# abhishekjoshi2/cuGP

Measured on AMD Instinct MI355X. Metric: GP log-lik+grad evals/sec (N=8192, D=10), higher is better.
Workload: dtype f64; 1 GPU; gp_loglik_grad_N8192_D10; experts=1, experts_per_gpu=1, overlap=True, full=False

## Files before the change

cugp_amd/capi.py:

```python
import ctypes as C
import os

import numpy as np

HERE = os.path.dirname(os.path.abspath(__file__))
LIB_PATH = os.path.join(HERE, "lib", "libcugp.so")

_dp = C.POINTER(C.c_double)
_ip = C.POINTER(C.c_int)
OBJECTIVE = C.CFUNCTYPE(None, C.c_void_p, _dp, _dp, _dp)
VALUE_FN = C.CFUNCTYPE(None, C.c_void_p, _dp, _dp)
GRADIENT_FN = C.CFUNCTYPE(None, C.c_void_p, _dp, _dp)
OBJECTIVE_N = C.CFUNCTYPE(None, C.c_void_p, _dp, C.c_int, _dp, _dp)

CUGP_OK = 0
CUGP_KERNEL_SE, CUGP_KERNEL_MATERN32, CUGP_KERNEL_MATERN52 = 0, 1, 2
CUGP_COMBINE_POE, CUGP_COMBINE_GPOE, CUGP_COMBINE_BCM, CUGP_COMBINE_RBCM = 0, 1, 2, 3
CUGP_COMBINE_REFERENCE = -1
CUGP_ERR_INVALID, CUGP_ERR_NOMEM, CUGP_ERR_DEVICE, CUGP_ERR_NODEVICE = -1, -2, -3, -4
ERR_NAMES = {-1: "CUGP_ERR_INVALID", -2: "CUGP_ERR_NOMEM", -3: "CUGP_ERR_DEVICE", -4: "CUGP_ERR_NODEVICE",
             -5: "CUGP_ERR_BUSY"}


class CugpError(RuntimeError):
# ... 129 lines not shown
    "cugp_bcm_create_split_ard_kernel": (C.c_int, [_dp, _dp, C.c_int, C.c_int, C.c_int, C.c_int, _ip, C.c_int,
                                                   C.POINTER(C.c_void_p)]),
    "cugp_bcm_num_hyper": (C.c_int, [C.c_void_p, _ip]),
    "cugp_bcm_set_loghyper_ard": (C.c_int, [C.c_void_p, _dp, C.c_int]),
    "cugp_bcm_get_loghyper_ard": (C.c_int, [C.c_void_p, _dp, C.c_int]),
    "cugp_bcm_loglik_grad_ard": (C.c_int, [C.c_void_p, _dp, _dp, C.c_int, _dp]),
    "cugp_bcm_loglik_grad_rows_ard": (C.c_int, [C.c_void_p, _dp, C.c_int]),
    "cugp_bcm_loglik_grad_rows_device_ard": (C.c_int, [C.c_void_p, C.c_void_p, _ip, C.c_int]),
    "cugp_bcm_loglik_grad_allgather_ard": (C.c_int, [C.c_void_p, C.c_void_p, C.c_int, C.c_int, _dp]),
    "cugp_bcm_cg_solve_ard": (C.c_int, [C.c_void_p, C.c_int, _dp, C.c_int, _ip]),
    "cugp_test_gemm_nt": (C.c_int, [C.c_int, C.c_int, C.c_int, _dp, _dp, _dp, C.c_int]),
    "cugp_mfma_peak_tflops": (C.c_int, [C.c_int, _dp]),
    "cugp_set_tuning": (C.c_int, [C.c_int, C.c_int]),
    "cugp_set_handle_tuning": (C.c_int, [C.c_void_p, C.c_int, C.c_int, C.c_int]),
    "cugp_get_handle_tuning": (C.c_int, [C.c_void_p, C.c_int, C.POINTER(C.c_int)]),
    "cugp_bench_la": (C.c_int, [C.c_int, C.c_int, C.c_int, C.c_int, _dp]),
    "cugp_bench_la_check": (C.c_int, [C.c_int, C.c_int, C.c_int, C.c_int, _dp, _dp]),
    "cugp_potrf_plan": (C.c_int, [C.c_int, C.c_int, C.c_int, C.c_int, _ip]),
    "cugp_potrf_plan_sub": (C.c_int, [C.c_int, C.c_int, C.c_int, C.c_int, C.c_int, _ip]),
}

_lib = None


def _share_torch_hip_runtime():
    import importlib.util
    import sys
    if "torch" in sys.modules or os.environ.get("CUGP_OWN_HIP_RUNTIME", "0") not in ("", "0"):
        return
    try:
# ... 43 lines not shown
```

cugp_amd/csrc/bcm.cpp:

```cpp
#include <cmath>
#include <cstdio>
#include <cstring>
#include <new>
#include <vector>

#include "../../include/cugp.h"
#include <hip/hip_runtime.h>

#include "group.h"

struct DeviceSet {
    int device = 0;
    std::vector<int> idx;
    cugp_group* group = nullptr;
    bool grouped_now = false;
    Scratch grad_rows;
    hipStream_t grad_stream = nullptr;
    std::vector<hipEvent_t> ev;
};

struct cugp_bcm {
    std::vector<DeviceSet> sets;
    std::vector<cugp_gp*> experts;
    std::vector<int> rows;
// ... 92 lines not shown
        if (rows[k] <= 0) { delete b; return CUGP_ERR_INVALID; }
        nmax = rows[k] > nmax ? rows[k] : nmax;
        nmin = rows[k] < nmin ? rows[k] : nmin;
    }
    const int tmax = (nmax + 127) / 128, tmin = (nmin + 127) / 128;
    const int pad_to = (tmax - tmin <= (tmin / 16 > 1 ? tmin / 16 : 1)) ? nmax : 0;
    const int nsets = ndev < nexperts ? ndev : nexperts;
    b->sets.resize(nsets);
    for (int s = 0; s < nsets; s++) b->sets[s].device = devices[s];
    for (int k = 0; k < nexperts; k++) {
        DeviceSet& ds = b->sets[k % nsets];
        cugp_gp* g = nullptr;
        int rc = ard ? cugp_create_ard_kernel(rows[k], d, ds.device, pad_to, kernel, &g)
                     : cugp_create_kernel(rows[k], d, ds.device, pad_to, kernel, &g);
        if (rc) { cugp_bcm_destroy(b); return rc; }
        cugp_mark_bcm_expert(g);
        if (nexperts > nsets) cugp_set_overlap(g, 0);
        b->experts.push_back(g);
        b->rows.push_back(rows[k]);
        ds.idx.push_back(k);
    }
    for (DeviceSet& ds : b->sets) {
        if (ds.idx.size() < 2 && !(nexperts > nsets)) continue;
        std::vector<cugp_gp*> mine;
        for (int k : ds.idx) mine.push_back(b->experts[k]);
        if (cugp_group_create(mine.data(), (int)mine.size(), &ds.group) != CUGP_OK) ds.group = nullptr;
    }
    *out = b;
    return CUGP_OK;
}

int bcm_create_split(const double* X, const double* y, int N, int D, int K, int ndev, const int* devices, int kernel,
                     bool ard, cugp_bcm** out)
// ... 796 lines not shown
```

cugp_amd/csrc/cugp_capi.cpp:

```cpp
#include <hip/hip_runtime.h>

#include <algorithm>
#include <atomic>
#include <cmath>
#include <cstdio>
#include <cstdlib>
#include <cstdint>
#include <cstring>
#include <mutex>
#include <string>
#include <vector>

#include "../../include/cugp.h"
#include "group.h"
#include "kernels.h"

using namespace cugp;

namespace {

thread_local std::string g_err;

int fail(int code, const char* what, hipError_t e = hipSuccess)
{
// ... 51 lines not shown
    unsigned* tickets = nullptr;
    double* dout = nullptr;
    double* hout = nullptr;
    int row = 8;
    double* hrows = nullptr;
    bool overlap = false;
    int gcap = 0;
};

struct cugp_gp {
    int n = 0, d = 0, npad = 0, nt = 0, device = 0;
    hipStream_t stream = nullptr;
    hipStream_t aux = nullptr;
    hipStream_t aux2 = nullptr;
    hipStream_t lq = nullptr;
    std::vector<hipEvent_t> bev;
    std::vector<hipEvent_t> oev;
    std::vector<hipEvent_t> lev;
    double *dX = nullptr, *dy = nullptr, *dA = nullptr, *dT = nullptr, *dU = nullptr, *dKinv = nullptr;
    double *dz = nullptr, *dalpha = nullptr, *dw = nullptr, *d16 = nullptr, *dlogdet = nullptr, *dpart = nullptr, *d64 = nullptr;
    double* dout = nullptr;
    unsigned* dtickets = nullptr;
    double* hout = nullptr;
    int nblocks_trace = 0;
    bool ard = false;
    int nh = 3;
    std::vector<double> theta = {0, 0, 0}, last_g = {NAN, NAN, NAN};
    int kernel = KERNEL_SE;
    bool have_data = false;
    bool factor_valid = false;
// ... 219 lines not shown
{
    if (g->bar_quota > 0) g_bar_used[g->device >= 0 && g->device < 64 ? g->device : 63].fetch_sub(g->bar_quota, std::memory_order_relaxed);
    g->bar_quota = -1;
}
int barrier_cap(cugp_gp* g)
{
    if (g->grp) return g->grp->gcap;
    const int share = barrier_share(g);
    return g->overlap && share >= 16 ? share / 2 : share;
}

int pipe_block(const cugp_gp* g, bool with_inverse)
{
    const bool overlap = g->grp ? g->grp->overlap : g->overlap;
    int w = (with_inverse && overlap) ? g->tune[TUNE_PIPE_BLOCK] : 0;
    if (w < 0) w = g->nt <= 8 ? 1 : ((g->nt + 8) / 16 > 2 ? (g->nt + 8) / 16 : 2);
    return w >= g->nt ? 0 : w;
}

struct TimedLaunch {
    cugp_gp* g; hipStream_t s; bool on, ext;
    TimedLaunch(cugp_gp* g_, hipStream_t s_, bool want, bool chain = false)
        : g(g_), s(s_), on(want && g_->kev_used + 2 <= (int)g_->kev.size()), ext(g_->prof >= 4)
    {
        if (!on) { if (chain) g->last_main = -1; return; }
        g->kev_prev[g->kev_used / 2] = chain ? g->last_main : -1;
        if (chain) g->last_main = g->kev_used / 2;
        if (g->prof >= 5) stamp_next_launch(g->dstamps + g->kev_used / 2);
        else if (ext) time_next_launch(g->kev[g->kev_used], g->kev[g->kev_used + 1]);
        else if (hipEventRecord(g->kev[g->kev_used], s) != hipSuccess) on = false;
    }
    ~TimedLaunch() { if (on && ext && timing_pending()) { time_next_launch(nullptr, nullptr); stamp_next_launch(nullptr); } }
// ... 584 lines not shown
    g->kernel = kernel;
    if (ard) { g->nh = d + 2; g->theta.assign(g->nh, 0.0); g->last_g.assign(g->nh, NAN); }
    const size_t nrow = ard ? (size_t)ARD_ROW_GRAD + g->nh : 8, ncol = g->nh;
    g->nt = ((n > npad_min ? n : npad_min) + TILE - 1) / TILE;
    g->npad = g->nt * TILE;
    g->nblocks_trace = trace_num_blocks(g->npad);
    *out = nullptr;
    {
        std::lock_guard<std::mutex> lk(g_tune_mu);
        tune_defaults_locked();
        for (int k = 0; k < TUNE_COUNT; k++) g->tune[k] = g_tune_default[k];
    }
    g_live[device < 64 ? device : 63].fetch_add(1, std::memory_order_relaxed);
    g->counted = true;
    hipError_t e = hipSetDevice(device);
    int plo = 0, phi = 0;
    if (e == hipSuccess && g->tune[TUNE_STREAM_PRIO] != 0) e = hipDeviceGetStreamPriorityRange(&plo, &phi);
    const int pmain = (g->tune[TUNE_STREAM_PRIO] & 1) ? phi : 0, pinv = (g->tune[TUNE_STREAM_PRIO] & 2) ? plo : 0;
    auto mkstream = [&](hipStream_t* s, int prio) {
        return g->tune[TUNE_STREAM_PRIO] != 0 ? hipStreamCreateWithPriority(s, hipStreamNonBlocking, prio)
                                             : hipStreamCreateWithFlags(s, hipStreamNonBlocking);
    };
    if (e == hipSuccess) e = mkstream(&g->stream, pmain);
    if (e == hipSuccess) e = mkstream(&g->aux, pinv);
    if (e == hipSuccess) e = mkstream(&g->aux2, pinv);
    if (e == hipSuccess) e = mkstream(&g->lq, pinv);
    for (std::vector<hipEvent_t>* v : {&g->bev, &g->oev, &g->lev}) {
        v->assign((size_t)g->nt + 2, nullptr);
        for (size_t i = 0; i < v->size() && e == hipSuccess; i++) e = hipEventCreateWithFlags(&(*v)[i], hipEventDisableTiming);
    }
    if (e == hipSuccess) e = hipMalloc((void**)&g->dX, (size_t)n * d * sizeof(double));
    if (e == hipSuccess) e = hipMalloc((void**)&g->dy, (size_t)g->npad * sizeof(double));
    if (e == hipSuccess) e = hipMalloc((void**)&g->dz, (size_t)g->npad * sizeof(double));
    if (e == hipSuccess) e = hipMalloc((void**)&g->dalpha, (size_t)g->npad * sizeof(double));
    if (e == hipSuccess) e = hipMalloc((void**)&g->dw, (size_t)g->npad * sizeof(double));
    if (e == hipSuccess) e = hipMalloc((void**)&g->d16, (size_t)g->nt * 8 * 256 * sizeof(double));
    if (e == hipSuccess) e = hipMalloc((void**)&g->d64, (size_t)g->nt * 8192 * sizeof(double));
    if (e == hipSuccess) e = hipMalloc((void**)&g->dlogdet, (size_t)g->nt * sizeof(double));
    if (e == hipSuccess) e = hipMalloc((void**)&g->dpart, (size_t)g->nblocks_trace * ncol * sizeof(double));
    if (e == hipSuccess) e = hipMalloc((void**)&g->dout, nrow * sizeof(double));
    if (e == hipSuccess) e = hipMalloc((void**)&g->dtickets, (size_t)ticket_count(g->nt) * sizeof(unsigned));
// ... 49 lines not shown
    for (hipEvent_t e : g->kev) (void)hipEventDestroy(e);
    for (std::vector<hipEvent_t>* v : {&g->bev, &g->oev, &g->lev})
        for (hipEvent_t e : *v)
            if (e) (void)hipEventDestroy(e);
    if (g->aux) (void)hipStreamDestroy(g->aux);
    if (g->aux2) (void)hipStreamDestroy(g->aux2);
    if (g->lq) (void)hipStreamDestroy(g->lq);
    if (g->stream) (void)hipStreamDestroy(g->stream);
    delete g;
    return CUGP_OK;
}

int cugp_set_overlap(cugp_gp* g, int enable)
{
    if (!g) return CUGP_ERR_INVALID;
    g->overlap = enable != 0;
    return CUGP_OK;
}

int cugp_dims(const cugp_gp* g, int* n, int* d, int* npad)
{
    if (!g) return CUGP_ERR_INVALID;
    if (n) *n = g->n;
    if (d) *d = g->d;
    if (npad) *npad = g->npad;
    return CUGP_OK;
}

static int set_data_common(cugp_gp* g, const double* X, const double* y, hipMemcpyKind kind)
{
    if (!g || !X || !y) return fail(CUGP_ERR_INVALID, "cugp_set_data: null argument");
    int rc;
    if ((rc = use_device(g))) return rc;
    if ((rc = fetch_eval(g))) return rc;
    HIPCHK(hipMemcpyAsync(g->dX, X, (size_t)g->n * g->d * sizeof(double), kind, g->stream));
    HIPCHK(hipMemsetAsync(g->dy, 0, (size_t)g->npad * sizeof(double), g->stream));
    HIPCHK(hipMemcpyAsync(g->dy, y, (size_t)g->n * sizeof(double), kind, g->stream));
    HIPCHK(hipStreamSynchronize(g->stream));
    g->have_data = true;
    g->factor_valid = g->inverse_valid = false;
    return CUGP_OK;
}

int cugp_set_data(cugp_gp* g, const double* X, const double* y) { return set_data_common(g, X, y, hipMemcpyHostToDevice); }

int cugp_set_data_device(cugp_gp* g, const double* dX, const double* dy)
{
    return set_data_common(g, dX, dy, hipMemcpyDeviceToDevice);
}
// ... 422 lines not shown

static int cov_factor_handle(cugp_gp* g, int tiles)
{
    int rc;
    if (!g->cov_f || g->cov_tiles < tiles) {
        HIPCHK(hipStreamSynchronize(g->stream));
        if (g->cov_f) (void)cugp_destroy(g->cov_f);
        g->cov_f = nullptr;
        g->cov_tiles = 0;
        cugp_gp* f = nullptr;
        if ((rc = cugp_create(tiles * TILE, 1, g->device, &f))) return rc;
        g_live[f->device < 64 ? f->device : 63].fetch_sub(1, std::memory_order_relaxed);
        f->counted = false;
        f->overlap = false;
        f->is_factor = true;
        if ((rc = ensure_factor_bufs(f))) { cugp_destroy(f); return rc; }
        g->cov_f = f;
        g->cov_tiles = tiles;
        if ((rc = use_device(g))) return rc;
    }
    return CUGP_OK;
}

static int predict_cov_device(cugp_gp* g, const double* Xt, int nt, bool with_noise, double jitter, double** dmean,
                              cugp_gp** fout)
{
    PredBufs pb;
    int rc;
    if ((rc = predict_device(g, Xt, nt, &pb))) return rc;
    TuneScope ts(g);
    const int tiles = (nt + TILE - 1) / TILE, ntpad = tiles * TILE;
// ... 209 lines not shown
    launch_trace(g->dX, g->n, d, g->npad, cf, g->dKinv, g->dalpha, g->dpart, s, {}, g->dz, g->dlogdet, g->dout, g->hout,
                 g->dtickets + 2 * g->nt);
    hipError_t e = hipGetLastError();
    if (e == hipSuccess) e = hipStreamSynchronize(s);
    if (e != hipSuccess) { (void)hipStreamSynchronize(s); return fail(CUGP_ERR_DEVICE, "cugp_append", e); }
    g->pev_valid = false;
    (void)read_result_row(g, g->hout, true);
    if (!std::isfinite(g->last_ll)) discard_eval(g);
    return CUGP_OK;
}

int cugp_mark_bcm_expert(cugp_gp* g)
{
    if (!g) return CUGP_ERR_INVALID;
    g->bcm_expert = true;
    return CUGP_OK;
}

int cugp_compute_K_train(cugp_gp* g, double* K)
{
    if (!g || !K) return CUGP_ERR_INVALID;
    if (!g->have_data) return fail(CUGP_ERR_INVALID, "no training data set");
    int rc;
    if ((rc = use_device(g))) return rc;
    if ((rc = fetch_eval(g))) return rc;
    if ((rc = ensure(&g->dA, (size_t)g->npad * g->npad))) return rc;
    g->factor_valid = g->inverse_valid = false;
    TuneScope ts(g);
    CovFn cf;
    if ((rc = cov_fn(g, g->stream, nullptr, &cf))) return rc;
    launch_kbuild(g->dX, g->n, g->d, g->npad, cf, g->dA, true, g->stream);
// ... 1010 lines not shown
    tune_defaults_locked();
    g_tune_default[key] = value;
    return CUGP_OK;
}

int cugp_set_handle_tuning(cugp_gp* g, int key, int value, int own)
{
    if (!g || key < 0 || key >= TUNE_COUNT) return CUGP_ERR_INVALID;
    int rc;
    if ((rc = fetch_eval(g))) return rc;
    g->tune_own[key] = own != 0;
    if (own && g->tune[key] != value) {
        g->tune[key] = value;
        if (key != TUNE_GRAPHS) g->cfg_epoch++;
    }
    return CUGP_OK;
}

int cugp_get_handle_tuning(cugp_gp* g, int key, int* value)
{
    if (!g || !value || key < 0 || key >= TUNE_COUNT) return CUGP_ERR_INVALID;
    sync_tuning(g);
    *value = g->tune[key];
    return CUGP_OK;
}

int cugp_potrf_plan(int nt, int P, int near, int kb, int out[5])
{
    int v[6];
    const int rc = cugp_potrf_plan_sub(nt, P, near, 1, kb, v);
    if (rc || !out) return rc ? rc : CUGP_ERR_INVALID;
// ... 139 lines not shown
    if (!experts || k <= 0 || !out) return CUGP_ERR_INVALID;
    for (int i = 0; i < k; i++)
        if (!experts[i] || experts[i]->npad != experts[0]->npad || experts[i]->d != experts[0]->d ||
            experts[i]->device != experts[0]->device)
            return CUGP_ERR_INVALID;
    for (int i = 0; i < k; i++)
        if (experts[i]->kernel != experts[0]->kernel)
            return fail(CUGP_ERR_INVALID, "cugp_group_create: the experts have different kernel kinds (one launch serves them all)");
    for (int i = 0; i < k; i++)
        if (experts[i]->ard != experts[0]->ard)
            return fail(CUGP_ERR_INVALID, "cugp_group_create: ARD and isotropic handles in one group (the experts of a group are all ARD or all isotropic)");
    cugp_group* gr = new (std::nothrow) cugp_group;
    if (!gr) return fail(CUGP_ERR_NOMEM, "host allocation");
    gr->experts.assign(experts, experts + k);
    for (cugp_gp* x : gr->experts) x->groups++;
    const int nt = experts[0]->nt;
    const bool ard = experts[0]->ard;
    const size_t row = ard ? (size_t)ARD_ROW_GRAD + experts[0]->nh : 8;
    gr->ctx.row = (int)row;
    hipError_t e = hipSetDevice(experts[0]->device);
    if (e == hipSuccess) e = hipMalloc((void**)&gr->dtab, (size_t)k * sizeof(ExpertPtrs));
    if (e == hipSuccess) e = hipMalloc((void**)&gr->ctx.tickets, (size_t)k * ticket_count(nt) * sizeof(unsigned));
    if (e == hipSuccess) e = hipMalloc((void**)&gr->ctx.dout, (size_t)k * row * sizeof(double));
    if (e == hipSuccess) e = hipHostMalloc((void**)&gr->ctx.hout, (size_t)k * 8 * sizeof(double), hipHostMallocDefault);
    if (e == hipSuccess) memset(gr->ctx.hout, 0, (size_t)k * 8 * sizeof(double));
    if (e == hipSuccess && ard) e = hipHostMalloc((void**)&gr->ctx.hrows, (size_t)k * row * sizeof(double), hipHostMallocDefault);
    if (e == hipSuccess && ard) memset(gr->ctx.hrows, 0, (size_t)k * row * sizeof(double));
    if (e != hipSuccess) {
        cugp_group_destroy(gr);
        return fail(e == hipErrorOutOfMemory ? CUGP_ERR_NOMEM : CUGP_ERR_DEVICE, "cugp_group_create", e);
// ... 254 lines not shown
```

cugp_amd/csrc/kernels.h:

```cpp
#pragma once
#ifndef CUGP_HOST_EMUL
#include <hip/hip_runtime.h>
#endif

namespace cugp {

constexpr int TILE = 128;

enum { TUNE_LAUUM_WM2_MAX = 0,
       TUNE_TRTRI_WM2_MAX = 1,
       TUNE_SYRK_REM_MAX = 2,
       TUNE_PIPE_BLOCK = 3,
       TUNE_BORDER_WM2_MAX = 4,
       TUNE_GRAPHS = 5,
       TUNE_GROUP_OVERLAP = 6,
       TUNE_GROUP_MAX_TILES = 7,
       TUNE_PANEL = 8,
       TUNE_NEAR_TILES = 9,
       TUNE_PANEL_MIN_NT = 10,
       TUNE_LAUUM_STREAM = 11,
       TUNE_FINALIZE_FUSE_MAX = 12,
       TUNE_SPLIT_REM_MAX = 13,
       TUNE_STEP_QUARTER_MAX = 14,
       TUNE_STREAM_PRIO = 15,
       TUNE_BARRIER_SPIN = 16,
       TUNE_SUBPANEL = 17,
       TUNE_ZFUSE = 18,
       TUNE_PRED_CHUNK = 19,
       TUNE_COV_SPLIT = 20,
       TUNE_COUNT = 21 };
extern const int g_tune_init[TUNE_COUNT];
extern thread_local const int* t_tune;
inline int tune(int key) { return t_tune[key]; }

enum { KERNEL_SE = 0, KERNEL_MATERN32 = 1, KERNEL_MATERN52 = 2, KERNEL_COUNT = 3 };

struct ExpertPtrs {
    double *A, *T, *U, *Kinv, *d16, *d64, *logdet, *y, *z, *alpha, *w, *part, *out;
    const double* X;
    unsigned* tickets;
    int n;
};
struct Batch {
    const ExpertPtrs* tab = nullptr;
    int count = 1;
// ... 154 lines not shown
```

cugp_amd/csrc/kernels.hip:

```cpp
#include "kernels.h"

#include <hip/hip_runtime.h>
#include <hip/hip_ext.h>

#include <cassert>
#include <cstdlib>

namespace cugp {

typedef double d4 __attribute__((ext_vector_type(4)));
typedef double d2 __attribute__((ext_vector_type(2)));

template <class T>
__device__ __forceinline__ T* GP(T* p)
{
    return (T*)(__attribute__((address_space(1))) T*)(unsigned long long)p;
}

#ifdef CUGP_WGTIMES
constexpr unsigned WGT_CAP = 1u << 19;
__device__ unsigned long long g_wgt[4 * WGT_CAP];
__device__ unsigned g_wgt_n;
struct WgTimer {
    unsigned long long t0, c0, tag;
// ... 426 lines not shown
                                                         int c0, int c1, int nfull, const ExpertPtrs* __restrict__ bt,
                                                         unsigned long long* stamp)
{
    LaunchStamp stamp_(stamp);
    if (bt) { L = GP(bt[blockIdx.y].A); T = GP(bt[blockIdx.y].T); U = GP(bt[blockIdx.y].U); }
    extern __shared__ __attribute__((aligned(16))) char smem[];
    WGT(wgt_, WGT_BORDER, a * 4 + step);
    if (WM == 2) {
        border_tile<2>(L, T, U, ld, a, w, step, c0, c1, blockIdx.x >> 2, blockIdx.x & 3, smem);
    } else if ((int)blockIdx.x < nfull) {
        border_tile<4>(L, T, U, ld, a, w, step, c0, c1, blockIdx.x, 0, smem);
    } else {
        const int y = blockIdx.x - nfull;
        border_tile<2>(L, T, U, ld, a, w, step, c0, c1, nfull + (y >> 2), y & 3, smem);
    }
}

__global__ __launch_bounds__(256, 2) void k_predict_gemm(const double* __restrict__ Ks, const double* __restrict__ T,
                                                         double* __restrict__ W, int ld, int ntt64, int n64,
                                                         unsigned long long* stamp, const ExpertPtrs* __restrict__ bt)
{
    LaunchStamp stamp_(stamp);
    if (bt) {
        const size_t off = (size_t)blockIdx.y * ntt64 * 64 * ld;
        T = GP(bt[blockIdx.y].T); Ks += off; W += off;
    }
    extern __shared__ __attribute__((aligned(16))) char smem[];
    const int tt = blockIdx.x % ntt64, p = blockIdx.x / ntt64;
#pragma unroll 1
    for (int h = 0; h < 2; h++) {
// ... 1101 lines not shown
        tile_accum_store<-1>(A + (size_t)i0 * ld + j0, ld, acc);
        return;
    }
    const int xg = blockIdx.x & 7;
    const int xq = nfull >> 3, xr = nfull & 7;
    const int tlin = (xg < xr ? xg * (xq + 1) : xr * (xq + 1) + (xg - xr) * xq) + (blockIdx.x >> 3);
    int ti, tj;
    trap_index(rev ? nfull - 1 - tlin : tlin, cb - ca, ti, tj);
    const int i0 = (ca + ti) * TILE, j0 = (ca + tj) * TILE;
    d4 acc[4][4];
    acc_zero(acc);
    tile_nt<false>(A + (size_t)i0 * ld, ld, A + (size_t)j0 * ld, ld, k0 * TILE, (k0 + kw) * TILE, acc, smem);
    tile_accum_store<-1>(A + (size_t)i0 * ld + j0, ld, acc);
}

__device__ __forceinline__ void trtri_diag_body(const double* __restrict__ A, int ld, int b,
                                                const double* __restrict__ d64, double* __restrict__ T,
                                                double* __restrict__ U, double* __restrict__ sm)
{
    const int t = threadIdx.x, wave = t >> 6;
    const double* Ab = A + (size_t)b * TILE * ld + b * TILE;
    const double* T00 = d64 + (size_t)b * 8192;
    const double* T11 = T00 + 4096;
    {
        const int r = t >> 4, c = t & 15;
        double v[NLT];
#pragma unroll
        for (int bi = 0; bi < NMT; bi++)
#pragma unroll
            for (int bj = 0; bj <= bi; bj++) {
// ... 810 lines not shown
void stamp_next_launch(unsigned long long* slot) { t_stamp = slot; }
bool timing_pending() { return t_ev0 != nullptr || t_stamp != nullptr; }
static inline unsigned long long* take_stamp() { unsigned long long* p = t_stamp; t_stamp = nullptr; return p; }
#define CUGP_LAUNCH(kernel, grid, block, lds, stream, ...)                                          \
    do {                                                                                            \
        if (t_ev0) {                                                                                \
            hipEvent_t e0_ = t_ev0, e1_ = t_ev1;                                                    \
            t_ev0 = t_ev1 = nullptr;                                                                \
            hipExtLaunchKernelGGL(kernel, grid, block, lds, stream, e0_, e1_, 0, __VA_ARGS__);      \
        } else {                                                                                    \
            hipLaunchKernelGGL(kernel, grid, block, lds, stream, __VA_ARGS__);                      \
        }                                                                                           \
    } while (0)

const int g_tune_init[TUNE_COUNT] = {768, 1200, 384, -1, 511, 1, 1, 1 << 20, 16, 500, 32, 1, 2100, 256, 1536, 0, 1 << 21, 1, 1, 0,
                                      1024};
thread_local const int* t_tune = g_tune_init;

static inline int tri_count(int n) { return n * (n + 1) / 2; }

static inline bool is_ard(const CovFn& cf)
{
    assert(!cf.ard || cf.hd);
    return cf.ard;
}

#define CUGP_COV_KERNEL(cf, stem)                                                                        \
    (is_ard(cf) ? ((cf).kind == KERNEL_MATERN32   ? stem<true, KERNEL_MATERN32>                          \
                   : (cf).kind == KERNEL_MATERN52 ? stem<true, KERNEL_MATERN52> : stem<true, KERNEL_SE>) \
                : ((cf).kind == KERNEL_MATERN32   ? stem<false, KERNEL_MATERN32>                         \
                   : (cf).kind == KERNEL_MATERN52 ? stem<false, KERNEL_MATERN52> : stem<false, KERNEL_SE>))
// ... 29 lines not shown
    int dev = 0;
    if (hipGetDevice(&dev) != hipSuccess || dev < 0 || dev > 63) dev = 63;
    if (g_attr_done >> dev & 1ull) return;
    hipError_t e = hipSuccess;
    auto attr = [&](const void* f, int bytes) {
        const hipError_t r = hipFuncSetAttribute(f, hipFuncAttributeMaxDynamicSharedMemorySize, bytes);
        if (r != hipSuccess && e == hipSuccess) e = r;
    };
    attr((const void*)k_potf2, POTF2_LDS);
    attr((const void*)k_syrk_step, STEP_LDS);
    attr((const void*)k_syrk_wide, GEMM_LDS);
    const void* gemm4[] = {(const void*)k_trtri_level<4>, (const void*)k_trtri_border<4>, (const void*)k_lauum<4>,
                           (const void*)k_test_gemm, (const void*)k_predict_cov<4>, (const void*)k_loo_product<4>,
                           (const void*)k_sparse_gram};
    for (const void* f : gemm4) attr(f, GEMM_LDS);
    attr((const void*)k_trtri_diag, TRTRI_LDS);
    attr((const void*)k_trtri_block, TRTRI_BLOCK_LDS);
    attr((const void*)k_trsm_inv64, TRSM_LDS);
    if (e != hipSuccess) { g_attr_err = e; return; }
    g_attr_done |= 1ull << dev;
}

int prepare_kernels() { set_big_lds(); return (int)g_attr_err; }

void launch_potf2(double* A, int ld, int kb, double* d16, double* d64, double* logdet_part, hipStream_t s, Batch bt)
{
    set_big_lds();
    hipLaunchKernelGGL(k_potf2, dim3(1, bt.count), dim3(256), POTF2_LDS, s, A, ld, kb, d16, d64, logdet_part, bt.tab);
}

// ... 58 lines not shown
    const int vec0 = NDIAGWG + nfull + 4 * (ntl - nfull);
    const unsigned nwg = vec0 + (zv ? m : 0);
    if (ks < 0 || ks > kb) ks = kb;
    if (kb + 1 - ks > SUBPANEL_MAX) return;
    CUGP_LAUNCH(k_syrk_step, bt.tab ? dim3(bt.count, nwg) : dim3(nwg), dim3(256), STEP_LDS, s, A, ld, kb, d16,
                       d64, logdet_part, tickets, nfull, wcol, ks, bt.tab, take_stamp(), vec0, zv, wv);
}

int launch_syrk_wide(double* A, int ld, int nt, int k0, int kw, int ca, int cb, int rev, hipStream_t s, Batch bt)
{
    if (cb > nt) cb = nt;
    if (ca >= cb || kw <= 0) return 0;
    set_big_lds();
    const int ntiles = trap_count(nt - ca, cb - ca);
    const int nfull = split_round(ntiles, bt.count);
    CUGP_LAUNCH(k_syrk_wide, dim3(nfull + 4 * (ntiles - nfull), bt.count), dim3(256), GEMM_LDS, s, A, ld, k0, kw, ca,
                       cb, ntiles, nfull, rev, bt.tab, take_stamp());
    return ntiles;
}

int launch_trtri_level(const double* L, double* T, double* U, int ld, int nt, int s, int step, hipStream_t st,
                       Batch bt, size_t off)
{
    int tiles = 0;
    for (int a0 = 0; a0 + s < nt; a0 += 2 * s) {
        int sb = nt - (a0 + s);
        if (sb > s) sb = s;
        tiles += s * sb;
    }
    if (tiles <= 0) return 0;
// ... 8 lines not shown
    return 4;
}

int launch_trtri_border1(const double* L, double* T, double* U, int ld, int ra, int rw, int c0, int c1,
                         hipStream_t st, Batch bt)
{
    const int tiles = c1 * rw;
    if (tiles <= 0) return 0;
    set_big_lds();
    if (tiles * bt.count <= tune(TUNE_BORDER_WM2_MAX)) {
        CUGP_LAUNCH(k_trtri_border<2>, dim3(tiles * 4, bt.count), dim3(256), Geo<2>::LDS, st, L, T, U, ld, ra, rw,
                           1, c0, c1, 0, bt.tab, take_stamp());
        return 2;
    }
    const int nfull = split_round(tiles, bt.count);
    CUGP_LAUNCH(k_trtri_border<4>, dim3(nfull + 4 * (tiles - nfull), bt.count), dim3(256), GEMM_LDS, st, L, T,
                       U, ld, ra, rw, 1, c0, c1, nfull, bt.tab, take_stamp());
    return 4;
}

int launch_trtri_border2(const double* L, double* T, double* U, int ld, int a, int w, hipStream_t st, Batch bt)
{
    const int tiles = a * w;
    if (tiles <= 0) return 0;
    set_big_lds();
    if (tiles * bt.count <= tune(TUNE_TRTRI_WM2_MAX)) {
        CUGP_LAUNCH(k_trtri_border<2>, dim3(tiles * 4, bt.count), dim3(256), Geo<2>::LDS, st, L, T, U, ld, a, w, 2,
                           0, 0, 0, bt.tab, take_stamp());
        return 2;
    }
    const int nfull = split_round(tiles, bt.count);
    CUGP_LAUNCH(k_trtri_border<4>, dim3(nfull + 4 * (tiles - nfull), bt.count), dim3(256), GEMM_LDS, st, L, T,
                       U, ld, a, w, 2, 0, 0, nfull, bt.tab, take_stamp());
    return 4;
}

int launch_lauum(const double* U, double* Kinv, int ld, int a, int w, hipStream_t s, Batch bt)
{
    set_big_lds();
    const int tiles = tri_count(a + w);
    if (tiles * bt.count <= tune(TUNE_LAUUM_WM2_MAX)) {
        CUGP_LAUNCH(k_lauum<2>, dim3(tiles * 4, bt.count), dim3(256), Geo<2>::LDS, s, U, Kinv, ld, a, w, 0, bt.tab, take_stamp());
        return 2;
    } else {
        const int nfull = a > 0 ? split_round(tiles, bt.count) : tiles;
        CUGP_LAUNCH(k_lauum<4>, dim3(nfull + 4 * (tiles - nfull), bt.count), dim3(256), GEMM_LDS, s, U, Kinv, ld,
                           a, w, nfull, bt.tab, take_stamp());
        return 4;
    }
}

void launch_predict_gemm(const double* Ks, const double* T, double* W, int ld, int ntt, int nt, hipStream_t s,
                         Batch bt)
{
    set_big_lds();
    CUGP_LAUNCH(k_predict_gemm, dim3(2 * ntt * nt, bt.count), dim3(256), Geo<2>::LDS, s, Ks, T, W, ld, 2 * ntt, 2 * nt,
                take_stamp(), bt.tab);
}

CovShape predict_cov_shape(int ntpad, int n)
// ... 381 lines not shown
```

cugp_amd/gp.py:

```python
import ctypes as C
import math

import numpy as np

from . import capi
from .capi import check, f64, ptr


KERNELS = {"se": capi.CUGP_KERNEL_SE, "matern32": capi.CUGP_KERNEL_MATERN32, "matern52": capi.CUGP_KERNEL_MATERN52}
KERNEL_NAMES = {v: k for k, v in KERNELS.items()}
ARD_KERNELS = {"matern32_ard": capi.CUGP_KERNEL_MATERN32, "matern52_ard": capi.CUGP_KERNEL_MATERN52}


COMBINE = {"poe": capi.CUGP_COMBINE_POE, "gpoe": capi.CUGP_COMBINE_GPOE, "bcm": capi.CUGP_COMBINE_BCM,
           "rbcm": capi.CUGP_COMBINE_RBCM}


def combine_mode(combine):
    if not isinstance(combine, str) or combine.lower() not in COMBINE:
        raise ValueError("combine must be None or one of %s, not %r" % (sorted(COMBINE), combine))
    return COMBINE[combine.lower()]


def prior_scalars(hp):
# ... 337 lines not shown
        return tr[: ne.value]

    def set_profiling(self, level):
        check(capi.lib().cugp_set_profiling(self._h, int(level)))

    def set_overlap(self, enable):
        check(capi.lib().cugp_set_overlap(self._h, 1 if enable else 0))

    def set_tuning(self, key, value, own=True):
        check(capi.lib().cugp_set_handle_tuning(self._h, int(key), int(value), 1 if own else 0))

    def get_tuning(self, key):
        v = C.c_int()
        check(capi.lib().cugp_get_handle_tuning(self._h, int(key), C.byref(v)))
        return v.value

    def phase_ms(self):
        ms = np.empty(6)
        check(capi.lib().cugp_get_phase_ms(self._h, ptr(ms)))
        return dict(zip(("kbuild", "potrf", "trtri", "lauum", "tail", "total"), ms.tolist()))

    def kernel_stats(self, reset=False, kind=0):
        s, n, f, dms = C.c_double(), C.c_longlong(), C.c_double(), C.c_double()
        check(capi.lib().cugp_get_kernel_stats_dispatch_ms(self._h, int(kind), C.byref(dms)))
        check(capi.lib().cugp_get_kernel_stats_kind(self._h, int(kind), C.byref(s), C.byref(n), C.byref(f),
                                                    1 if reset else 0))
        return {"sum_ms": s.value, "launches": n.value, "flop": f.value, "disp_ms": dms.value}


class SparseGP:
# ... 485 lines not shown
```

include/cugp.h:

```cpp
#ifndef CUGP_H
#define CUGP_H

#ifdef __cplusplus
extern "C" {
#endif

#define CUGP_OK 0
#define CUGP_ERR_INVALID (-1)
#define CUGP_ERR_NOMEM (-2)
#define CUGP_ERR_DEVICE (-3)
#define CUGP_ERR_NODEVICE (-4)
#define CUGP_ERR_BUSY (-5)

typedef struct cugp_gp cugp_gp;
typedef struct cugp_bcm cugp_bcm;

int cugp_version(void);
const char *cugp_build_id(void);
const char *cugp_last_error(void);
int cugp_device_count(int *count);

int cugp_create(int n, int d, int device, cugp_gp **out);
int cugp_create_padded(int n, int d, int device, int npad_min, cugp_gp **out);
int cugp_destroy(cugp_gp *gp);
// ... 170 lines not shown
int cugp_bcm_set_loghyper_ard(cugp_bcm *b, const double *hp, int nh);
int cugp_bcm_get_loghyper_ard(const cugp_bcm *b, double *hp, int nh);
int cugp_bcm_loglik_grad_ard(cugp_bcm *b, double *ll, double *g, int nh, double *per_expert_ll );
int cugp_bcm_loglik_grad_rows_ard(cugp_bcm *b, double *rows, int nh);
int cugp_bcm_loglik_grad_rows_device_ard(cugp_bcm *b, double *dev_rows, const int *slot, int nh);
int cugp_bcm_loglik_grad_allgather_ard(cugp_bcm *b, cugp_comm *c, int per, int nh, double *rows_out);
int cugp_bcm_cg_solve_ard(cugp_bcm *b, int budget, double *trace, int trace_cap, int *nevals);

int cugp_test_gemm_nt(int m, int n, int k, const double *A, const double *B, double *C, int device);
int cugp_mfma_peak_tflops(int device, double *tflops);
int cugp_bench_la(int op, int n, int device, int reps, double *ms);
int cugp_bench_la_check(int op, int n, int device, int reps, double *ms, double *logdet);
int cugp_set_tuning(int key, int value);
int cugp_set_handle_tuning(cugp_gp *gp, int key, int value, int own);
int cugp_get_handle_tuning(cugp_gp *gp, int key, int *value);
int cugp_potrf_plan(int nt, int P, int near_tiles, int kb, int out[5]);
int cugp_potrf_plan_sub(int nt, int P, int near_tiles, int S, int kb, int out[6]);

#ifdef __cplusplus
}
#endif
#endif
```

Baseline: 91.58 evals/s.

## Prioritize the factor chain stream and widen the inverse pipeline block for single GPs

Stream creation moves into a reusable apply_stream_prio helper. For a standalone overlapped GP with at least 64 tiles, the main (factorization) stream now gets high priority by default, and streams are recreated whenever overlap, the expert role or the tuning changes. The default pipeline block width for non-grouped GPs now comes from cugp_pipe_block_for, which gives larger blocks for big tile counts. The change also adds 512-thread, 8-wave variants of the syrk, trtri-border and lauum kernels behind TUNE_WAVES8, which is off by default. The aim is to keep the critical Cholesky chain ahead of the overlapped inverse work, at the cost of recreating streams and possibly starving the inverse work.

```diff
diff --git a/cugp_amd/capi.py b/cugp_amd/capi.py
--- a/cugp_amd/capi.py
+++ b/cugp_amd/capi.py
@@ -167,6 +167,8 @@
     "cugp_set_tuning": (C.c_int, [C.c_int, C.c_int]),
     "cugp_set_handle_tuning": (C.c_int, [C.c_void_p, C.c_int, C.c_int, C.c_int]),
     "cugp_get_handle_tuning": (C.c_int, [C.c_void_p, C.c_int, C.POINTER(C.c_int)]),
+    "cugp_chain_first": (C.c_int, [C.c_void_p, _ip]),
+    "cugp_pipe_block_for": (C.c_int, [C.c_int]),
     "cugp_bench_la": (C.c_int, [C.c_int, C.c_int, C.c_int, C.c_int, _dp]),
     "cugp_bench_la_check": (C.c_int, [C.c_int, C.c_int, C.c_int, C.c_int, _dp, _dp]),
     "cugp_potrf_plan": (C.c_int, [C.c_int, C.c_int, C.c_int, C.c_int, _ip]),
diff --git a/cugp_amd/csrc/bcm.cpp b/cugp_amd/csrc/bcm.cpp
--- a/cugp_amd/csrc/bcm.cpp
+++ b/cugp_amd/csrc/bcm.cpp
@@ -130,9 +130,10 @@
         int rc = ard ? cugp_create_ard_kernel(rows[k], d, ds.device, pad_to, kernel, &g)
                      : cugp_create_kernel(rows[k], d, ds.device, pad_to, kernel, &g);
         if (rc) { cugp_bcm_destroy(b); return rc; }
-        cugp_mark_bcm_expert(g);
-        if (nexperts > nsets) cugp_set_overlap(g, 0);
         b->experts.push_back(g);
+        rc = cugp_mark_bcm_expert(g);
+        if (!rc && nexperts > nsets) rc = cugp_set_overlap(g, 0);
+        if (rc) { cugp_bcm_destroy(b); return rc; }
         b->rows.push_back(rows[k]);
         ds.idx.push_back(k);
     }
diff --git a/cugp_amd/csrc/cugp_capi.cpp b/cugp_amd/csrc/cugp_capi.cpp
--- a/cugp_amd/csrc/cugp_capi.cpp
+++ b/cugp_amd/csrc/cugp_capi.cpp
@@ -89,6 +89,8 @@
     hipStream_t aux = nullptr;
     hipStream_t aux2 = nullptr;
     hipStream_t lq = nullptr;
+    int prio_main = 0, prio_inv = 0;
+    bool chain_first = false;
     std::vector<hipEvent_t> bev;
     std::vector<hipEvent_t> oev;
     std::vector<hipEvent_t> lev;
@@ -338,8 +340,51 @@
 {
     const bool overlap = g->grp ? g->grp->overlap : g->overlap;
     int w = (with_inverse && overlap) ? g->tune[TUNE_PIPE_BLOCK] : 0;
-    if (w < 0) w = g->nt <= 8 ? 1 : ((g->nt + 8) / 16 > 2 ? (g->nt + 8) / 16 : 2);
+    if (w < 0) w = !g->grp && !g->bcm_expert ? cugp_pipe_block_for(g->nt)
+                                            : g->nt <= 8 ? 1 : ((g->nt + 8) / 16 > 2 ? (g->nt + 8) / 16 : 2);
     return w >= g->nt ? 0 : w;
+}
+
+bool want_chain_first(const cugp_gp* g)
+{
+    const int v = g->tune[TUNE_STREAM_PRIO];
+    if (v != 0) return (v & 4) == 0 && (v & 1) != 0;
+    return !g->bcm_expert && g->groups == 0 && !g->is_factor && g->overlap && g->tune[TUNE_PIPE_BLOCK] != 0 &&
+           g->nt >= g->tune[TUNE_PRIO_MIN_NT];
+}
+
+int apply_stream_prio(cugp_gp* g)
+{
+    const int v = g->tune[TUNE_STREAM_PRIO];
+    const bool first = want_chain_first(g), inv_low = (v & 4) == 0 && (v & 2) != 0;
+    int plo = 0, phi = 0;
+    if (first || inv_low) HIPCHK(hipDeviceGetStreamPriorityRange(&plo, &phi));
+    const int pmain = first ? phi : 0, pinv = inv_low ? plo : 0;
+    hipStream_t* const all[4] = {&g->stream, &g->aux, &g->aux2, &g->lq};
+    if (g->stream && pmain == g->prio_main && pinv == g->prio_inv) return CUGP_OK;
+    hipStream_t fresh[4] = {nullptr, nullptr, nullptr, nullptr};
+    hipError_t e = hipSuccess;
+    for (int i = 0; i < 4 && e == hipSuccess; i++) {
+        const int p = i == 0 ? pmain : pinv;
+        e = pmain == 0 && pinv == 0 ? hipStreamCreateWithFlags(&fresh[i], hipStreamNonBlocking)
+                                    : hipStreamCreateWithPriority(&fresh[i], hipStreamNonBlocking, p);
+    }
+    for (int i = 0; i < 4 && e == hipSuccess; i++)
+        if (*all[i]) e = hipStreamSynchronize(*all[i]);
+    if (e != hipSuccess) {
+        for (hipStream_t s : fresh)
+            if (s) (void)hipStreamDestroy(s);
+        return fail(CUGP_ERR_DEVICE, "apply_stream_prio: the handle keeps the streams it had", e);
+    }
+    for (int i = 0; i < 4; i++) {
+        if (*all[i]) (void)hipStreamDestroy(*all[i]);
+        *all[i] = fresh[i];
+    }
+    g->prio_main = pmain;
+    g->prio_inv = pinv;
+    g->chain_first = first;
+    g->cfg_epoch++;
+    return CUGP_OK;
 }
 
 struct TimedLaunch {
@@ -954,17 +999,7 @@
     g_live[device < 64 ? device : 63].fetch_add(1, std::memory_order_relaxed);
     g->counted = true;
     hipError_t e = hipSetDevice(device);
-    int plo = 0, phi = 0;
-    if (e == hipSuccess && g->tune[TUNE_STREAM_PRIO] != 0) e = hipDeviceGetStreamPriorityRange(&plo, &phi);
-    const int pmain = (g->tune[TUNE_STREAM_PRIO] & 1) ? phi : 0, pinv = (g->tune[TUNE_STREAM_PRIO] & 2) ? plo : 0;
-    auto mkstream = [&](hipStream_t* s, int prio) {
-        return g->tune[TUNE_STREAM_PRIO] != 0 ? hipStreamCreateWithPriority(s, hipStreamNonBlocking, prio)
-                                             : hipStreamCreateWithFlags(s, hipStreamNonBlocking);
-    };
-    if (e == hipSuccess) e = mkstream(&g->stream, pmain);
-    if (e == hipSuccess) e = mkstream(&g->aux, pinv);
-    if (e == hipSuccess) e = mkstream(&g->aux2, pinv);
-    if (e == hipSuccess) e = mkstream(&g->lq, pinv);
+    if (e == hipSuccess && apply_stream_prio(g) != CUGP_OK) e = hipErrorUnknown;
     for (std::vector<hipEvent_t>* v : {&g->bev, &g->oev, &g->lev}) {
         v->assign((size_t)g->nt + 2, nullptr);
         for (size_t i = 0; i < v->size() && e == hipSuccess; i++) e = hipEventCreateWithFlags(&(*v)[i], hipEventDisableTiming);
@@ -1044,8 +1079,10 @@
 int cugp_set_overlap(cugp_gp* g, int enable)
 {
     if (!g) return CUGP_ERR_INVALID;
+    int rc;
+    if ((rc = use_device(g)) || (rc = fetch_eval(g))) return rc;
     g->overlap = enable != 0;
-    return CUGP_OK;
+    return apply_stream_prio(g);
 }
 
 int cugp_dims(const cugp_gp* g, int* n, int* d, int* npad)
@@ -1063,6 +1100,8 @@
     int rc;
     if ((rc = use_device(g))) return rc;
     if ((rc = fetch_eval(g))) return rc;
+    sync_tuning(g);
+    if ((rc = apply_stream_prio(g))) return rc;
     HIPCHK(hipMemcpyAsync(g->dX, X, (size_t)g->n * g->d * sizeof(double), kind, g->stream));
     HIPCHK(hipMemsetAsync(g->dy, 0, (size_t)g->npad * sizeof(double), g->stream));
     HIPCHK(hipMemcpyAsync(g->dy, y, (size_t)g->n * sizeof(double), kind, g->stream));
@@ -1515,7 +1554,7 @@
         f->counted = false;
         f->overlap = false;
         f->is_factor = true;
-        if ((rc = ensure_factor_bufs(f))) { cugp_destroy(f); return rc; }
+        if ((rc = apply_stream_prio(f)) || (rc = ensure_factor_bufs(f))) { cugp_destroy(f); return rc; }
         g->cov_f = f;
         g->cov_tiles = tiles;
         if ((rc = use_device(g))) return rc;
@@ -1755,7 +1794,9 @@
 {
     if (!g) return CUGP_ERR_INVALID;
     g->bcm_expert = true;
-    return CUGP_OK;
+    int rc;
+    if ((rc = use_device(g)) || (rc = fetch_eval(g))) return rc;
+    return apply_stream_prio(g);
 }
 
 int cugp_compute_K_train(cugp_gp* g, double* K)
@@ -2796,7 +2837,27 @@
         g->tune[key] = value;
         if (key != TUNE_GRAPHS) g->cfg_epoch++;
     }
-    return CUGP_OK;
+    if (key != TUNE_STREAM_PRIO && key != TUNE_PRIO_MIN_NT && key != TUNE_PIPE_BLOCK) return CUGP_OK;
+    if (!own) sync_tuning(g);
+    if ((rc = use_device(g))) return rc;
+    return apply_stream_prio(g);
+}
+
+int cugp_chain_first(const cugp_gp* g, int* on)
+{
+    if (!g || !on) return fail(CUGP_ERR_INVALID, "cugp_chain_first: null argument");
+    *on = g->chain_first ? 1 : 0;
+    return CUGP_OK;
+}
+
+int cugp_pipe_block_for(int nt)
+{
+    if (nt <= 8) return 1;
+    int w = (nt + 8) / 16;
+    if (w < 2) w = 2;
+    if (nt >= 60 && w < 5) w = 5;
+    if (nt >= 72 && w < 8) w = 8;
+    return w > 16 ? 16 : w;
 }
 
 int cugp_get_handle_tuning(cugp_gp* g, int key, int* value)
@@ -2966,6 +3027,11 @@
     if (!gr) return fail(CUGP_ERR_NOMEM, "host allocation");
     gr->experts.assign(experts, experts + k);
     for (cugp_gp* x : gr->experts) x->groups++;
+    for (cugp_gp* x : gr->experts)
+        if (hipSetDevice(x->device) != hipSuccess || fetch_eval(x) != CUGP_OK || apply_stream_prio(x) != CUGP_OK) {
+            cugp_group_destroy(gr);
+            return fail(CUGP_ERR_DEVICE, "cugp_group_create: the experts' streams");
+        }
     const int nt = experts[0]->nt;
     const bool ard = experts[0]->ard;
     const size_t row = ard ? (size_t)ARD_ROW_GRAD + experts[0]->nh : 8;
diff --git a/cugp_amd/csrc/kernels.h b/cugp_amd/csrc/kernels.h
--- a/cugp_amd/csrc/kernels.h
+++ b/cugp_amd/csrc/kernels.h
@@ -28,7 +28,9 @@
        TUNE_ZFUSE = 18,
        TUNE_PRED_CHUNK = 19,
        TUNE_COV_SPLIT = 20,
-       TUNE_COUNT = 21 };
+       TUNE_PRIO_MIN_NT = 21,
+       TUNE_WAVES8 = 22,
+       TUNE_COUNT = 23 };
 extern const int g_tune_init[TUNE_COUNT];
 extern thread_local const int* t_tune;
 inline int tune(int key) { return t_tune[key]; }
diff --git a/cugp_amd/csrc/kernels.hip b/cugp_amd/csrc/kernels.hip
--- a/cugp_amd/csrc/kernels.hip
+++ b/cugp_amd/csrc/kernels.hip
@@ -464,6 +464,165 @@
         const int y = blockIdx.x - nfull;
         border_tile<2>(L, T, U, ld, a, w, step, c0, c1, nfull + (y >> 2), y & 3, smem);
     }
+}
+
+template <bool NEGA>
+__device__ __forceinline__ void tile_nt8(const double* __restrict__ Ag, int lda, const double* __restrict__ Bg, int ldb,
+                                         int kbeg, int kend, d4 (&acc)[2][4], char* smem)
+{
+    typedef Geo<4> G;
+    const int t = opaque_tid();
+    const int lane = t & 63, wave = t >> 6;
+    const int wr = wave >> 1, wc = wave & 1;
+    const int srow = t >> 3, skp = t & 7;
+    const double* ag = Ag + (size_t)srow * lda + 2 * skp;
+    const double* bg = Bg + (size_t)srow * ldb + 2 * skp;
+    d2 ra[2], rb[2];
+    int wa[2], wb[2];
+#pragma unroll
+    for (int q = 0; q < 2; q++) {
+        wa[q] = skp * G::PLANE + (srow + 64 * q) * 16;
+        wb[q] = G::OPER + skp * G::PLANE + bpos<4>(srow + 64 * q) * 16;
+    }
+    const int fr = lane & 15, fk = lane >> 4;
+    const int abase = (fk >> 1) * G::PLANE + (wr * 32 + fr) * 16 + (fk & 1) * 8;
+    const int bbase = G::OPER + (fk >> 1) * G::PLANE + (wc * 64 + fr) * 16 + (fk & 1) * 8;
+    const int nk = (kend - kbeg) / BK;
+    if (nk <= 0) return;
+#pragma unroll
+    for (int q = 0; q < 2; q++) {
+        ra[q] = *(const d2*)(ag + (size_t)(64 * q) * lda + kbeg);
+        rb[q] = *(const d2*)(bg + (size_t)(64 * q) * ldb + kbeg);
+    }
+#pragma unroll
+    for (int q = 0; q < 2; q++) {
+        *(d2*)(smem + wa[q]) = NEGA ? -ra[q] : ra[q];
+        *(d2*)(smem + wb[q]) = rb[q];
+    }
+    __syncthreads();
+#define CUGP_STAGE8(HALF, MORE, KNEXT)                                                              \
+    do {                                                                                            \
+        const char* cur_ = smem + (HALF) * G::STAGE;                                                \
+        char* nxt_ = smem + (1 - (HALF)) * G::STAGE;                                                \
+        const bool more_ = (MORE);                                                                  \
+        if (more_) {                                                                                \
+            const int k_ = (KNEXT);                                                                 \
+            _Pragma("unroll") for (int q = 0; q < 2; q++) {                                         \
+                ra[q] = *(const d2*)(ag + (size_t)(64 * q) * lda + k_);                             \
+                rb[q] = *(const d2*)(bg + (size_t)(64 * q) * ldb + k_);                             \
+            }                                                                                       \
+        }                                                                                           \
+        _Pragma("unroll") for (int kk = 0; kk < BK / 4; kk++) {                                     \
+            double a[2], b[4];                                                                      \
+            _Pragma("unroll") for (int m = 0; m < 2; m++) a[m] = *(const double*)(cur_ + abase + kk * 2 * G::PLANE + m * 256); \
+            _Pragma("unroll") for (int n = 0; n < 4; n++) b[n] = *(const double*)(cur_ + bbase + kk * 2 * G::PLANE + n * 256); \
+            _Pragma("unroll") for (int m = 0; m < 2; m++)                                           \
+                _Pragma("unroll") for (int n = 0; n < 4; n++)                                       \
+                    acc[m][n] = __builtin_amdgcn_mfma_f64_16x16x4f64(a[m], b[n], acc[m][n], 0, 0, 0); \
+        }                                                                                           \
+        if (more_) {                                                                                \
+            _Pragma("unroll") for (int q = 0; q < 2; q++) {                                         \
+                *(d2*)(nxt_ + wa[q]) = NEGA ? -ra[q] : ra[q];                                       \
+                *(d2*)(nxt_ + wb[q]) = rb[q];                                                       \
+            }                                                                                       \
+        }                                                                                           \
+        __syncthreads();                                                                            \
+    } while (0)
+    int kt = 0;
+    for (; kt + 1 < nk; kt += 2) {
+        CUGP_STAGE8(0, true, kbeg + (kt + 1) * BK);
+        CUGP_STAGE8(1, kt + 2 < nk, kbeg + (kt + 2) * BK);
+    }
+    if (kt < nk) CUGP_STAGE8(0, false, 0);
+#undef CUGP_STAGE8
+}
+
+template <int SIGN>
+__device__ __forceinline__ void tile_out8(double* __restrict__ C, int ldc, const d4 (&acc)[2][4])
+{
+    const int tid = opaque_tid();
+    const int lane = tid & 63, wave = tid >> 6;
+    const int wr = wave >> 1, wc = wave & 1;
+#pragma unroll
+    for (int m = 0; m < 2; m++) {
+        double* const c0 = C + (size_t)(wr * 32 + m * 16 + (lane >> 4)) * ldc + wc * 64 + 2 * (lane & 15);
+        d2 v[4][2];
+        if (SIGN != 0) {
+#pragma unroll
+            for (int r = 0; r < 4; r++)
+#pragma unroll
+                for (int np = 0; np < 2; np++) v[r][np] = *(const d2*)(c0 + (size_t)(4 * r) * ldc + np * 32);
+        }
+#pragma unroll
+        for (int r = 0; r < 4; r++)
+#pragma unroll
+            for (int np = 0; np < 2; np++) {
+                d2* dst = (d2*)(c0 + (size_t)(4 * r) * ldc + np * 32);
+                if (SIGN == 0) *dst = (d2){acc[m][2 * np][r], acc[m][2 * np + 1][r]};
+                else if (SIGN > 0) *dst = (d2){v[r][np][0] + acc[m][2 * np][r], v[r][np][1] + acc[m][2 * np + 1][r]};
+                else *dst = (d2){v[r][np][0] - acc[m][2 * np][r], v[r][np][1] - acc[m][2 * np + 1][r]};
+            }
+    }
+}
+
+__device__ __forceinline__ void acc_zero8(d4 (&acc)[2][4])
+{
+#pragma unroll
+    for (int m = 0; m < 2; m++)
+#pragma unroll
+        for (int n = 0; n < 4; n++) acc[m][n] = (d4){0.0, 0.0, 0.0, 0.0};
+}
+
+__global__ __launch_bounds__(512, 4) void k_lauum8(const double* __restrict__ U, double* __restrict__ Kinv, int ld, int a,
+                                                   int w, const ExpertPtrs* __restrict__ bt, unsigned long long* stamp)
+{
+    LaunchStamp stamp_(stamp);
+    if (bt) { U = GP(bt[blockIdx.y].U); Kinv = GP(bt[blockIdx.y].Kinv); }
+    extern __shared__ __attribute__((aligned(16))) char smem[];
+    int ti, tj;
+    tri_index(blockIdx.x, ti, tj);
+    double* C = Kinv + (size_t)(ti * TILE) * ld + tj * TILE;
+    d4 acc[2][4];
+    acc_zero8(acc);
+    tile_nt8<false>(U + (size_t)(ti * TILE) * ld, ld, U + (size_t)(tj * TILE) * ld, ld, (ti < a ? a : ti) * TILE,
+                    (a + w) * TILE, acc, smem);
+    if (ti < a) tile_out8<1>(C, ld, acc);
+    else tile_out8<0>(C, ld, acc);
+}
+
+__global__ __launch_bounds__(256, 2) void k_lauum_rest(const double* __restrict__ U, double* __restrict__ Kinv, int ld,
+                                                       int a, int w, int x0, const ExpertPtrs* __restrict__ bt)
+{
+    if (bt) { U = GP(bt[blockIdx.y].U); Kinv = GP(bt[blockIdx.y].Kinv); }
+    extern __shared__ __attribute__((aligned(16))) char smem[];
+    lauum_tile<2>(U, Kinv, ld, a, w, x0 + (blockIdx.x >> 2), blockIdx.x & 3, smem);
+}
+
+__global__ __launch_bounds__(512, 4) void k_trtri_border8(const double* __restrict__ L, double* __restrict__ T,
+                                                          const double* __restrict__ U, int ld, int a, int w, int c0,
+                                                          int c1, const ExpertPtrs* __restrict__ bt,
+                                                          unsigned long long* stamp)
+{
+    LaunchStamp stamp_(stamp);
+    if (bt) { L = GP(bt[blockIdx.y].A); T = GP(bt[blockIdx.y].T); U = GP(bt[blockIdx.y].U); }
+    extern __shared__ __attribute__((aligned(16))) char smem[];
+    const int tj = blockIdx.x / w, ti = a + blockIdx.x % w;
+    double* W = T + (size_t)(tj * TILE) * ld + ti * TILE;
+    d4 acc[2][4];
+    acc_zero8(acc);
+    tile_nt8<false>(U + (size_t)(tj * TILE) * ld, ld, L + (size_t)(ti * TILE) * ld, ld, (tj > c0 ? tj : c0) * TILE,
+                    c1 * TILE, acc, smem);
+    if (tj < c0) tile_out8<1>(W, ld, acc);
+    else tile_out8<0>(W, ld, acc);
+}
+
+__global__ __launch_bounds__(256, 2) void k_trtri_border_rest(const double* __restrict__ L, double* __restrict__ T,
+                                                              double* __restrict__ U, int ld, int a, int w, int c0,
+                                                              int c1, int x0, const ExpertPtrs* __restrict__ bt)
+{
+    if (bt) { L = GP(bt[blockIdx.y].A); T = GP(bt[blockIdx.y].T); U = GP(bt[blockIdx.y].U); }
+    extern __shared__ __attribute__((aligned(16))) char smem[];
+    border_tile<2>(L, T, U, ld, a, w, 1, c0, c1, x0 + (blockIdx.x >> 2), blockIdx.x & 3, smem);
 }
 
 __global__ __launch_bounds__(256, 2) void k_predict_gemm(const double* __restrict__ Ks, const double* __restrict__ T,
@@ -1595,6 +1754,43 @@
     tile_accum_store<-1>(A + (size_t)i0 * ld + j0, ld, acc);
 }
 
+__global__ __launch_bounds__(512, 4) void k_syrk_wide8(double* __restrict__ A, int ld, int k0, int kw, int ca, int cb,
+                                                       int rev, const ExpertPtrs* __restrict__ bt,
+                                                       unsigned long long* stamp)
+{
+    LaunchStamp stamp_(stamp);
+    if (bt) A = GP(bt[blockIdx.y].A);
+    extern __shared__ __attribute__((aligned(16))) char smem[];
+    __builtin_amdgcn_s_setprio(1);
+    const int nfull = gridDim.x;
+    const int xg = blockIdx.x & 7;
+    const int xq = nfull >> 3, xr = nfull & 7;
+    const int tlin = (xg < xr ? xg * (xq + 1) : xr * (xq + 1) + (xg - xr) * xq) + (blockIdx.x >> 3);
+    int ti, tj;
+    trap_index(rev ? nfull - 1 - tlin : tlin, cb - ca, ti, tj);
+    const int i0 = (ca + ti) * TILE, j0 = (ca + tj) * TILE;
+    d4 acc[2][4];
+    acc_zero8(acc);
+    tile_nt8<false>(A + (size_t)i0 * ld, ld, A + (size_t)j0 * ld, ld, k0 * TILE, (k0 + kw) * TILE, acc, smem);
+    tile_out8<-1>(A + (size_t)i0 * ld + j0, ld, acc);
+}
+
+__global__ __launch_bounds__(256, 2) void k_syrk_wide_rest(double* __restrict__ A, int ld, int k0, int kw, int ca, int cb,
+                                                           int x0, const ExpertPtrs* __restrict__ bt)
+{
+    if (bt) A = GP(bt[blockIdx.y].A);
+    extern __shared__ __attribute__((aligned(16))) char smem[];
+    __builtin_amdgcn_s_setprio(1);
+    const int y = blockIdx.x;
+    int ti, tj;
+    trap_index(x0 + (y >> 2), cb - ca, ti, tj);
+    const int i0 = (ca + ti) * TILE + ((y >> 1) & 1) * 64, j0 = (ca + tj) * TILE + (y & 1) * 64;
+    d4 acc[2][2];
+    acc_zero(acc);
+    tile_nt<false>(A + (size_t)i0 * ld, ld, A + (size_t)j0 * ld, ld, k0 * TILE, (k0 + kw) * TILE, acc, smem);
+    tile_accum_store<-1>(A + (size_t)i0 * ld + j0, ld, acc);
+}
+
 __device__ __forceinline__ void trtri_diag_body(const double* __restrict__ A, int ld, int b,
                                                 const double* __restrict__ d64, double* __restrict__ T,
                                                 double* __restrict__ U, double* __restrict__ sm)
@@ -2435,7 +2631,7 @@
     } while (0)
 
 const int g_tune_init[TUNE_COUNT] = {768, 1200, 384, -1, 511, 1, 1, 1 << 20, 16, 500, 32, 1, 2100, 256, 1536, 0, 1 << 21, 1, 1, 0,
-                                      1024};
+                                      1024, 64, 0};
 thread_local const int* t_tune = g_tune_init;
 
 static inline int tri_count(int n) { return n * (n + 1) / 2; }
@@ -2495,6 +2691,7 @@
                            (const void*)k_test_gemm, (const void*)k_predict_cov<4>, (const void*)k_loo_product<4>,
                            (const void*)k_sparse_gram};
     for (const void* f : gemm4) attr(f, GEMM_LDS);
+    for (const void* f : {(const void*)k_syrk_wide8, (const void*)k_lauum8, (const void*)k_trtri_border8}) attr(f, GEMM_LDS);
     attr((const void*)k_trtri_diag, TRTRI_LDS);
     attr((const void*)k_trtri_block, TRTRI_BLOCK_LDS);
     attr((const void*)k_trsm_inv64, TRSM_LDS);
@@ -2583,6 +2780,14 @@
     set_big_lds();
     const int ntiles = trap_count(nt - ca, cb - ca);
     const int nfull = split_round(ntiles, bt.count);
+    if (tune(TUNE_WAVES8) != 0 && nfull > 0) {
+        CUGP_LAUNCH(k_syrk_wide8, dim3(nfull, bt.count), dim3(512), GEMM_LDS, s, A, ld, k0, kw, ca, cb, rev, bt.tab,
+                    take_stamp());
+        if (ntiles > nfull)
+            hipLaunchKernelGGL(k_syrk_wide_rest, dim3(4 * (ntiles - nfull), bt.count), dim3(256), Geo<2>::LDS, s, A, ld, k0,
+                               kw, ca, cb, nfull, bt.tab);
+        return ntiles;
+    }
     CUGP_LAUNCH(k_syrk_wide, dim3(nfull + 4 * (ntiles - nfull), bt.count), dim3(256), GEMM_LDS, s, A, ld, k0, kw, ca,
                        cb, ntiles, nfull, rev, bt.tab, take_stamp());
     return ntiles;
@@ -2621,6 +2826,14 @@
         return 2;
     }
     const int nfull = split_round(tiles, bt.count);
+    if (tune(TUNE_WAVES8) != 0 && nfull > 0) {
+        CUGP_LAUNCH(k_trtri_border8, dim3(nfull, bt.count), dim3(512), GEMM_LDS, st, L, T, U, ld, ra, rw, c0, c1, bt.tab,
+                    take_stamp());
+        if (tiles > nfull)
+            hipLaunchKernelGGL(k_trtri_border_rest, dim3(4 * (tiles - nfull), bt.count), dim3(256), Geo<2>::LDS, st, L, T,
+                               U, ld, ra, rw, c0, c1, nfull, bt.tab);
+        return 4;
+    }
     CUGP_LAUNCH(k_trtri_border<4>, dim3(nfull + 4 * (tiles - nfull), bt.count), dim3(256), GEMM_LDS, st, L, T,
                        U, ld, ra, rw, 1, c0, c1, nfull, bt.tab, take_stamp());
     return 4;
@@ -2651,6 +2864,13 @@
         return 2;
     } else {
         const int nfull = a > 0 ? split_round(tiles, bt.count) : tiles;
+        if (tune(TUNE_WAVES8) != 0 && nfull > 0) {
+            CUGP_LAUNCH(k_lauum8, dim3(nfull, bt.count), dim3(512), GEMM_LDS, s, U, Kinv, ld, a, w, bt.tab, take_stamp());
+            if (tiles > nfull)
+                hipLaunchKernelGGL(k_lauum_rest, dim3(4 * (tiles - nfull), bt.count), dim3(256), Geo<2>::LDS, s, U, Kinv, ld,
+                                   a, w, nfull, bt.tab);
+            return 4;
+        }
         CUGP_LAUNCH(k_lauum<4>, dim3(nfull + 4 * (tiles - nfull), bt.count), dim3(256), GEMM_LDS, s, U, Kinv, ld,
                            a, w, nfull, bt.tab, take_stamp());
         return 4;
diff --git a/cugp_amd/gp.py b/cugp_amd/gp.py
--- a/cugp_amd/gp.py
+++ b/cugp_amd/gp.py
@@ -375,6 +375,11 @@
         v = C.c_int()
         check(capi.lib().cugp_get_handle_tuning(self._h, int(key), C.byref(v)))
         return v.value
+
+    def chain_first(self):
+        v = C.c_int()
+        check(capi.lib().cugp_chain_first(self._h, C.byref(v)))
+        return bool(v.value)
 
     def phase_ms(self):
         ms = np.empty(6)
diff --git a/include/cugp.h b/include/cugp.h
--- a/include/cugp.h
+++ b/include/cugp.h
@@ -208,6 +208,8 @@
 int cugp_set_tuning(int key, int value);
 int cugp_set_handle_tuning(cugp_gp *gp, int key, int value, int own);
 int cugp_get_handle_tuning(cugp_gp *gp, int key, int *value);
+int cugp_chain_first(const cugp_gp *gp, int *on);
+int cugp_pipe_block_for(int nt);
 int cugp_potrf_plan(int nt, int P, int near_tiles, int kb, int out[5]);
 int cugp_potrf_plan_sub(int nt, int P, int near_tiles, int S, int kb, int out[6]);
 
```

Result: faster. 92.89 evals/s (median of 6 runs) (+1.4%).
